# gattia/pyfocusr

Measured on AMD Instinct MI355X. Metric: lowest-k eigenpairs/sec + KNN-correspondence wall-clock, 250k-vertex mesh pair k=5, higher is better.
Workload: dtype f64

## Files before the change

### pyfocusr_amd/csrc/pf_eigs.hip

```cpp
#include <math.h>

#include <algorithm>
#include <vector>

#include "pf_internal.h"
#include "pf_krylov.h"
#include "pf_launch.h"

namespace {

struct DeviceOps final : pfk::Ops {
    pf_graph* g;
    explicit DeviceOps(pf_graph* graph) : g(graph) {}
    int64_t n() const override { return g->n; }
    int64_t n_isolated() const override { return g->n_isolated; }
    int32_t n_components() const override { return g->n_components; }
    int32_t n_oneway() const override { return g->n_oneway; }
    bool symmetric() const override { return g->is_symmetric; }
    double spectral_bound() const override { return g->spectral_bound; }
    int ws_ensure(int32_t slots) override { return pf_ws_ensure(g, slots); }
    int lock_nulls(int32_t op, int32_t* locked) override { return pf_lock_null_vectors(g, op, locked); }
    int orth_strict(bool on) override { return pf_orth_strict(g, on ? 1 : 0); }
    int orth_always_twice(bool on, bool strict_otherwise) override { return pf_orth_strict(g, on ? 2 : (strict_otherwise ? 1 : 0)); }
    int orth_device_passes(bool on) override { return pf_orth_device_passes(g, on ? 1 : 0); }
// ... 14 lines not shown
    }
    int combine2(int32_t src_first, int32_t m, const double* Y, int32_t k, int32_t dst_first, int32_t src_first2, int32_t dst_first2) override {
        return pf_combine2(g, src_first, m, Y, k, dst_first, src_first2, dst_first2);
    }
    int copy(int32_t src, int32_t dst, int32_t count) override { return pf_ws_copy(g, src, dst, count); }
    int spmv_multi(int32_t op, int32_t src_first, int32_t dst_first, int32_t count) override {
        return pf_spmv_multi(g, op, src_first, dst_first, count);
    }
    int gram(int32_t first_a, int32_t count_a, int32_t first_b, int32_t count_b, double* out) override {
        return pf_gram(g, first_a, count_a, first_b, count_b, out);
    }
    int resnorms(int32_t ax_first, int32_t x_first, const double* lam, int32_t count, double* out) override {
        return pf_resnorms(g, ax_first, x_first, lam, count, out);
    }
    int gram_begin(int32_t first_a, int32_t count_a, int32_t first_b, int32_t count_b, bool self_b) override {
        PF_TRY(pf_gram_begin(g, first_a, count_a, first_b, count_b, 0));
        return self_b ? pf_gram_begin(g, first_b, count_b, first_b, count_b, 1) : PF_OK;
    }
    bool orth_split(int32_t first2, int32_t split) override { return pf_orth_split(g, first2, split) == PF_OK; }
    int gram_end(double* out) override { return pf_small_end(g, out); }
    int resnorms_begin(int32_t ax_first, int32_t x_first, const double* lam, int32_t count) override {
        return pf_resnorms_begin(g, ax_first, x_first, lam, count);
    }
    int resnorms_end(double* out) override { return pf_small_end(g, out); }
    int orth_begin_pair(pfk::Ops& other, const int32_t* o) override {
        return pf_orth_begin2(g, o[0], o[1], o[2], o[3], static_cast<DeviceOps&>(other).g, o[4], o[5], o[6], o[7]);
    }
    int cheb_pair(pfk::Ops& other, const int32_t* ci, const double* cd) override {
        return pf_cheb2(g, ci[0], ci[1], ci[2], ci[3], cd[0], cd[1], cd[2], static_cast<DeviceOps&>(other).g, ci[4], ci[5], ci[6], ci[7], cd[3],
                        cd[4], cd[5]);
    }
    int orth_cheb_pair(pfk::Ops& other, const int32_t* orth, const int32_t* ci, const double* cd) override {
// ... 102 lines not shown
```

### pyfocusr_amd/csrc/pf_eigsort.hip

```cpp
#include <float.h>
#include <string.h>

#include <vector>

#include "pf_internal.h"

extern "C" int pf_knn1_blocks(pf_ctx* c, const double* ref_block, int64_t n_ref, int32_t ref_stride, const double* qry_block, int64_t n_qry,
                              int32_t qry_stride, int32_t d, const int32_t* col_ref, const double* scale_ref, const int32_t* col_qry,
                              const double* scale_qry, int64_t* idx_out, double* d2_out);

namespace {

constexpr int ES_SORT_THREADS = 1024;
constexpr int ES_MAX_SAMPLES = 16384;
constexpr int ES_RED_THREADS = 256;

__global__ __launch_bounds__(PF_BLOCK) void k_es_gather(const double* __restrict__ fin, int32_t fc, const double* __restrict__ pts,
                                                        const int64_t* __restrict__ rows, int64_t m, int32_t k,
                                                        const int32_t* __restrict__ col, const double* __restrict__ sign,
                                                        double* __restrict__ vals, double* __restrict__ raw) {
    const int64_t e = (int64_t)blockIdx.x * PF_BLOCK + threadIdx.x;
    if (e >= m * (k + 3)) return;
    const int64_t c = e / m, r = e - c * m;
    if (c < k) vals[c * m + r] = fin[rows[r] * fc + col[c]] * sign[c];
    else raw[r * 3 + (c - k)] = pts[rows[r] * 3 + (c - k)];
}

__global__ __launch_bounds__(ES_RED_THREADS) void k_es_minmax(const double* __restrict__ raw, int64_t m, double* __restrict__ lohi) {
    __shared__ double slo[ES_RED_THREADS], shi[ES_RED_THREADS];
    const int c = blockIdx.x;
    double lo = INFINITY, hi = -INFINITY;
    for (int64_t r = threadIdx.x; r < m; r += ES_RED_THREADS) {
        const double v = raw[r * 3 + c];
        lo = v < lo ? v : lo;
        hi = v > hi ? v : hi;
    }
    slo[threadIdx.x] = lo;
    shi[threadIdx.x] = hi;
    __syncthreads();
    for (int s = ES_RED_THREADS / 2; s > 0; s >>= 1) {
        if (threadIdx.x < s) {
            slo[threadIdx.x] = slo[threadIdx.x + s] < slo[threadIdx.x] ? slo[threadIdx.x + s] : slo[threadIdx.x];
            shi[threadIdx.x] = shi[threadIdx.x + s] > shi[threadIdx.x] ? shi[threadIdx.x + s] : shi[threadIdx.x];
        }
        __syncthreads();
    }
    if (threadIdx.x == 0) {
        lohi[c] = slo[0];
        lohi[3 + c] = shi[0];
    }
}

__global__ __launch_bounds__(PF_BLOCK) void k_es_normalize(const double* __restrict__ raw, const double* __restrict__ lohi, int64_t m,
                                                           double* __restrict__ out) {
    const int64_t e = (int64_t)blockIdx.x * PF_BLOCK + threadIdx.x;
    if (e >= m * 3) return;
    const int c = (int)(e % 3);
    out[e] = (raw[e] - lohi[c]) / (lohi[3 + c] - lohi[c]);
}

__global__ __launch_bounds__(ES_SORT_THREADS) void k_es_sort_log(const double* __restrict__ vals_t, const double* __restrict__ vals_s,
                                                                 int64_t mt, int64_t ms, int32_t k, double* __restrict__ lt,
                                                                 double* __restrict__ ls, double* __restrict__ lsf) {
    extern __shared__ double buf[];
    const int b = blockIdx.x;
    const int64_t m = b < k ? mt : ms;
    int n_pow2 = 2;
    while (n_pow2 < m) n_pow2 <<= 1;
    const double* src = b < k ? vals_t + (int64_t)b * m : vals_s + (int64_t)(b - k) * m;
    for (int i = threadIdx.x; i < n_pow2; i += ES_SORT_THREADS) buf[i] = i < m ? src[i] : INFINITY;
    __syncthreads();
    for (int size = 2; size <= n_pow2; size <<= 1) {
        for (int stride = size >> 1; stride > 0; stride >>= 1) {
            for (int t = threadIdx.x; t < n_pow2 / 2; t += ES_SORT_THREADS) {
                const int pos = 2 * t - (t & (stride - 1));
                const double a = buf[pos], c = buf[pos + stride];
                const bool up = (pos & size) == 0;
                if ((a > c) == up) {
                    buf[pos] = c;
                    buf[pos + stride] = a;
                }
            }
            __syncthreads();
        }
    }
    const double eps = DBL_EPSILON;
    if (b < k) {
        for (int64_t i = threadIdx.x; i < m; i += ES_SORT_THREADS) lt[(int64_t)b * m + i] = log(buf[i] + 0.5 + eps);
    } else {
        const int64_t o = (int64_t)(b - k) * m;
        for (int64_t i = threadIdx.x; i < m; i += ES_SORT_THREADS) {
            ls[o + i] = log(buf[i] + 0.5 + eps);
            lsf[o + i] = log(-buf[m - 1 - i] + 0.5 + eps);
        }
    }
}

__device__ __forceinline__ double es_block_sum(double v, double* sh) {
    sh[threadIdx.x] = v;
    __syncthreads();
    for (int s = ES_RED_THREADS / 2; s > 0; s >>= 1) {
        if (threadIdx.x < s) sh[threadIdx.x] += sh[threadIdx.x + s];
        __syncthreads();
    }
    const double r = sh[0];
    __syncthreads();
    return r;
}

// ... 12 lines not shown
            const double len = (double)(to - from) * unit;
            acc += len * fabs(t - ls[(int64_t)j * ms + b]);
            accf += len * fabs(t - lsf[(int64_t)j * ms + b]);
        }
    }
    acc = es_block_sum(acc, sh);
    accf = es_block_sum(accf, sh);
    if (threadIdx.x == 0) {
        out[i * k + j] = acc;
        out[k * k + i * k + j] = accf;
    }
}

__global__ __launch_bounds__(ES_RED_THREADS) void k_es_spatial(const double* __restrict__ vals_t, const double* __restrict__ vals_s,
                                                               const int64_t* __restrict__ idx, int64_t m, int64_t ms, int32_t k,
                                                               double* __restrict__ out) {
    __shared__ double sh[ES_RED_THREADS];
    const int i = blockIdx.x / k, j = blockIdx.x - i * k;
    double a = 0.0, f = 0.0;
    for (int64_t r = threadIdx.x; r < m; r += ES_RED_THREADS) {
        const int64_t nn = idx[r];
        const double t = vals_t[(int64_t)i * m + r], s = (nn >= 0 && nn < ms) ? vals_s[(int64_t)j * ms + nn] : NAN;
        const double d0 = s - t, d1 = -s - t;
        a += d0 * d0;
        f += d1 * d1;
    }
    a = es_block_sum(a, sh);
    f = es_block_sum(f, sh);
    if (threadIdx.x == 0) {
        out[2 * k * k + i * k + j] = sqrt(a) / (double)m;
        out[3 * k * k + i * k + j] = sqrt(f) / (double)m;
    }
}

}

// ... 24 lines not shown

    const size_t head = sizeof(int64_t) * (size_t)(mt + ms);
    const size_t small = ((sizeof(int32_t) * 2 * k + 7) & ~(size_t)7) + sizeof(double) * 2 * k;
    std::vector<unsigned char> host(head + small);
    memcpy(host.data(), rows_t, sizeof(int64_t) * (size_t)mt);
    memcpy(host.data() + sizeof(int64_t) * (size_t)mt, rows_s, sizeof(int64_t) * (size_t)ms);
    int32_t* hcol = reinterpret_cast<int32_t*>(host.data() + head);
    double* hsign = reinterpret_cast<double*>(host.data() + head + ((sizeof(int32_t) * 2 * k + 7) & ~(size_t)7));
    for (int32_t i = 0; i < k; ++i) {
        hcol[i] = col_t[i];
        hcol[k + i] = col_s[i];
        hsign[i] = sign_t[i];
        hsign[k + i] = sign_s[i];
    }
    const size_t kt = (size_t)k * (size_t)mt, ks = (size_t)k * (size_t)ms;
    const size_t doubles = 2 * kt + 3 * ks + 6 * (size_t)(mt + ms) + 12 + 4 * (size_t)k * k;
    unsigned char* d = nullptr;
    const size_t up_bytes = (host.size() + 7) & ~(size_t)7, out_bytes = sizeof(double) * 4 * (size_t)k * k;
    unsigned char* pin = nullptr;
    PF_TRY(pf_pinned_scratch(c, up_bytes + out_bytes, reinterpret_cast<void**>(&pin)));
    memcpy(pin, host.data(), host.size());
    PF_HIP(pf_malloc(st, (void**)&d, up_bytes + sizeof(double) * doubles));
    int rc = PF_OK;
    do {
        auto fail = [&](hipError_t e) {
            if (e == hipSuccess) return false;
            pf_set_error("pf_eigsort_costs: %s", hipGetErrorString(e));
            rc = PF_E_HIP;
            return true;
        };
        if ((rc = pf_copy_by_kernel(st, pin, d, up_bytes)) != PF_OK) break;
        const int64_t* d_rows_t = reinterpret_cast<const int64_t*>(d);
        const int64_t* d_rows_s = d_rows_t + mt;
        const int32_t* d_col = reinterpret_cast<const int32_t*>(d + head);
        const double* d_sign = reinterpret_cast<const double*>(d + head + ((sizeof(int32_t) * 2 * k + 7) & ~(size_t)7));
        double* base = reinterpret_cast<double*>(d + up_bytes);
        double* vals_t = base;
        double* vals_s = vals_t + kt;
        double* raw_t = vals_s + ks;
        double* raw_s = raw_t + 3 * mt;
        double* norm_t = raw_s + 3 * ms;
        double* norm_s = norm_t + 3 * mt;
        double* lohi = norm_s + 3 * ms;
        double* lt = lohi + 12;
        double* ls = lt + kt;
        double* lsf = ls + ks;
        double* d_out = lsf + ks;
        k_es_gather<<<pf_blocks(mt * (k + 3)), PF_BLOCK, 0, st>>>(gt->final_vecs, gt->final_count, gt->pts, d_rows_t, mt, k, d_col, d_sign,
                                                                  vals_t, raw_t);
        k_es_gather<<<pf_blocks(ms * (k + 3)), PF_BLOCK, 0, st>>>(gs->final_vecs, gs->final_count, gs->pts, d_rows_s, ms, k, d_col + k,
                                                                  d_sign + k, vals_s, raw_s);
        k_es_minmax<<<3, ES_RED_THREADS, 0, st>>>(raw_t, mt, lohi);
        k_es_minmax<<<3, ES_RED_THREADS, 0, st>>>(raw_s, ms, lohi + 6);
        k_es_normalize<<<pf_blocks(3 * mt), PF_BLOCK, 0, st>>>(raw_t, lohi, mt, norm_t);
        k_es_normalize<<<pf_blocks(3 * ms), PF_BLOCK, 0, st>>>(raw_s, lohi + 6, ms, norm_s);
        k_es_sort_log<<<(unsigned)(2 * k), ES_SORT_THREADS, sort_lds, st>>>(vals_t, vals_s, mt, ms, k, lt, ls, lsf);
        k_es_w1<<<(unsigned)(k * k), ES_RED_THREADS, 0, st>>>(lt, ls, lsf, mt, ms, k, d_out);
        if (fail(hipGetLastError())) break;
        const int32_t cols3[3] = {0, 1, 2};
        const double ones3[3] = {1.0, 1.0, 1.0};
        rc = pf_knn1_blocks(c, norm_s, ms, 3, norm_t, mt, 3, 3, cols3, ones3, cols3, ones3, idx_out, nullptr);
        if (rc != PF_OK) break;
        k_es_spatial<<<(unsigned)(k * k), ES_RED_THREADS, 0, st>>>(vals_t, vals_s, c->knn_idx.p, mt, ms, k, d_out);
        if (fail(hipGetLastError())) break;
        if ((rc = pf_copy_by_kernel(st, d_out, pin + up_bytes, out_bytes)) != PF_OK) break;
        if (fail(hipStreamSynchronize(st))) break;
        memcpy(out, pin + up_bytes, out_bytes);
    } while (0);
    if (rc != PF_OK) (void)hipStreamSynchronize(st);
    pf_free(st, d);
    return rc;
}
```

### pyfocusr_amd/csrc/pf_internal.h

```cpp
#pragma once
#include <hip/hip_runtime.h>
#include <stdint.h>
#include <atomic>
#include <map>
#include <mutex>
#include <type_traits>
#include <unordered_map>
#include <vector>

#include "../../include/pyfocusr_hip.h"
#include "pf_scratch.h"

void pf_set_error(const char* fmt, ...);

#define PF_HIP(call)                                                                          \
    do {                                                                                      \
        hipError_t e_ = (call);                                                               \
        if (e_ != hipSuccess) {                                                               \
            pf_set_error("%s:%d %s: %s", __FILE__, __LINE__, #call, hipGetErrorString(e_));   \
            (void)hipGetLastError();  \
            return PF_E_HIP;                                                                  \
        }                                                                                     \
    } while (0)

// ... 296 lines not shown

int pf_graph_finish_general(pf_graph* g, const double* d_pts);

int pf_exclusive_scan_i32(hipStream_t st, const int32_t* in, int32_t* out, int64_t n);
int pf_exclusive_scan_i64(hipStream_t st, const int64_t* in, int64_t* out, int64_t n);

int pf_reduce_ensure(pf_graph* g, int32_t count);

int pf_compute_order(pf_graph* g, const double* d_pts, int32_t* d_overflow = nullptr);
int pf_morton_order(pf_graph* g, const double* d_pts, int32_t* d_overflow);

static inline int32_t pf_window_rows(int64_t n_pad) { return n_pad <= 262144 ? 1024 : (n_pad <= 524288 ? 2048 : 4096); }

int pf_knn1_device(pf_ctx* c, const double* ref_block, int64_t n_ref, int32_t ref_stride, const double* qry_block, int64_t n_qry,
                   int32_t qry_stride, int32_t d);

int pf_knn_extent(hipStream_t st, const double* pts, int64_t n, int32_t d, unsigned long long* ext);

constexpr int PF_KNN_TREE_MIN_D = 7;
int pf_knn_tree_run(pf_ctx* c);

int pf_gram_begin(pf_graph* g, int32_t first_a, int32_t count_a, int32_t first_b, int32_t count_b, int32_t append);
int pf_resnorms_begin(pf_graph* g, int32_t ax_first, int32_t x_first, const double* lam, int32_t count);
int pf_small_end(pf_graph* g, double* out);
int pf_combine2(pf_graph* g, int32_t src_first, int32_t m, const double* Y, int32_t k, int32_t dst_first, int32_t src_first2,
                int32_t dst_first2);

struct pf_persist_args {
    pf_graph* g;
    const double* vals;
    const double* src;
    double* dst;
    int32_t degree;
    double c, e, rho;
};
int pf_persist_cheb(const pf_persist_args* a, const pf_persist_args* b , int* done, double* lds_bytes ,
                    bool first_try = true );
// ... 13 lines not shown
```

### pyfocusr_amd/csrc/pf_knn.hip

```cpp
#include <hipcub/hipcub.hpp>

#include <string.h>

#include <algorithm>

#include "pf_internal.h"
#include "pf_wave.h"

namespace {

constexpr int KNN_LDS_DOUBLES = 4096;

struct KnnGrid {
    int a0, a1;
    int r0, r1;
    double lo0, lo1;
    double s0, s1;
};

__device__ __forceinline__ int cell_of(double x, double lo, double scale, int r) {
    const double t = (x - lo) * scale;
    return t > 0.0 ? (t >= (double)r ? r - 1 : (int)t) : 0;
}

// ... 853 lines not shown
           int64_t* idx_out, double* d2_out) {
    PF_TRY(knn_upload_k(c, ref, n_ref, qry, n_qry, d, k));
    PF_TRY(pf_knn_run(c));
    return pf_knn_download(c, idx_out, d2_out);
}

int pf_knn1(pf_ctx* c, const double* ref, int64_t n_ref, const double* qry, int64_t n_qry, int32_t d, int64_t* idx_out,
            double* d2_out) {
    PF_TRY(pf_knn_upload(c, ref, n_ref, qry, n_qry, d));
    PF_TRY(pf_knn_run(c));
    return pf_knn_download(c, idx_out, d2_out);
}

static int knn1_blocks_run(pf_ctx* c, const double* ref_block, int64_t n_ref, int32_t ref_stride, const double* qry_block, int64_t n_qry,
                           int32_t qry_stride, int32_t d, const int32_t* col_ref, const double* scale_ref, const int32_t* col_qry,
                           const double* scale_qry) {
    PF_TRY(knn_prepare(c, n_ref, n_qry, d, 1));
    hipStream_t st = c->stream;
    CoordMap mr{}, mq{};
    for (int32_t k = 0; k < d; ++k) {
        mr.col[k] = col_ref[k], mr.scale[k] = scale_ref[k];
        mq.col[k] = col_qry[k], mq.scale[k] = scale_qry[k];
    }
    k_coords_from_final<<<pf_blocks(n_ref * d), PF_BLOCK, 0, st>>>(ref_block, n_ref, ref_stride, d, mr, c->knn_ref.p);
    k_coords_from_final<<<pf_blocks(n_qry * d), PF_BLOCK, 0, st>>>(qry_block, n_qry, qry_stride, d, mq, c->knn_qry.p);
    PF_HIP(hipGetLastError());
    c->knn_ready = true;
    return pf_knn_run(c);
}

int pf_knn1_blocks(pf_ctx* c, const double* ref_block, int64_t n_ref, int32_t ref_stride, const double* qry_block, int64_t n_qry,
                   int32_t qry_stride, int32_t d, const int32_t* col_ref, const double* scale_ref, const int32_t* col_qry,
                   const double* scale_qry, int64_t* idx_out, double* d2_out) {
    PF_CHECK(c && ref_block && qry_block && col_ref && scale_ref && col_qry && scale_qry && idx_out, PF_E_ARG,
             "pf_knn1_blocks: NULL argument");
    PF_CHECK(d >= 1 && d <= 16 && ref_stride >= 1 && qry_stride >= 1, PF_E_ARG, "pf_knn1_blocks: d = %d / strides out of range", d);
    for (int32_t k = 0; k < d; ++k)
        PF_CHECK(col_ref[k] >= 0 && col_ref[k] < ref_stride && col_qry[k] >= 0 && col_qry[k] < qry_stride, PF_E_ARG,
                 "pf_knn1_blocks: column %d out of range", k);
    PF_TRY(knn1_blocks_run(c, ref_block, n_ref, ref_stride, qry_block, n_qry, qry_stride, d, col_ref, scale_ref, col_qry, scale_qry));
    return pf_knn_download(c, idx_out, d2_out);
// ... 22 lines not shown
int pf_knn_extent(hipStream_t st, const double* pts, int64_t n, int32_t d, unsigned long long* ext) {
    PF_HIP(hipMemsetAsync(ext, 0xff, 16 * sizeof(unsigned long long), st));
    PF_HIP(hipMemsetAsync(ext + 16, 0x00, 16 * sizeof(unsigned long long), st));
    k_extent<<<256, PF_BLOCK, 0, st>>>(pts, n, d, ext);
    return PF_OK;
}

int pf_knn1_device(pf_ctx* c, const double* ref_block, int64_t n_ref, int32_t ref_stride, const double* qry_block, int64_t n_qry,
                   int32_t qry_stride, int32_t d) {
    PF_CHECK(c && ref_block && qry_block && d >= 1 && d <= 16 && d <= ref_stride && d <= qry_stride, PF_E_ARG, "pf_knn1_device: bad argument");
    int32_t col[16];
    double one[16];
    for (int32_t k = 0; k < 16; ++k) col[k] = k, one[k] = 1.0;
    return knn1_blocks_run(c, ref_block, n_ref, ref_stride, qry_block, n_qry, qry_stride, d, col, one, col, one);
}
```

### pyfocusr_amd/csrc/pf_operator.hip

```cpp
#include <math.h>
#include <stdlib.h>
#include <string.h>

#include <algorithm>
#include <atomic>
#include <map>
#include <mutex>
#include <vector>

#include "pf_internal.h"
#include "pf_launch.h"

namespace {

#ifndef PF_OP_BLOCK
#define PF_OP_BLOCK 256
#endif
struct OpArgs {
    const int64_t* slice_ptr;
    const int32_t* scol;
    const double* sval;
    const double* diag;
    const double* x;
    const double* prev;
// ... 635 lines not shown
    const int64_t lo = (int64_t)blockIdx.x * PF_DOT_CHUNK;
    const int64_t hi = lo + PF_DOT_CHUNK < n_pad ? lo + PF_DOT_CHUNK : n_pad;
    double s = 0.0;
    for (int64_t i = lo + threadIdx.x; i < hi; i += PF_BLOCK) {
        const double r = ax[i] - lam * x[i];
        s += r * r;
    }
#pragma unroll
    for (int off = PF_WAVE / 2; off > 0; off >>= 1) s += __shfl_down(s, off, PF_WAVE);
    if ((threadIdx.x & (PF_WAVE - 1)) == 0) red[threadIdx.x / PF_WAVE] = s;
    __syncthreads();
    if (threadIdx.x == 0) partial[blockIdx.x] = (red[0] + red[1]) + (red[2] + red[3]);
}

__global__ __launch_bounds__(PF_BLOCK) void k_gram_partial(const double* __restrict__ ws, int64_t n_pad, int32_t first_a, int32_t first_b,
                                                           int32_t count_b, int64_t n_chunks, double* __restrict__ partial) {
    __shared__ double red[PF_BLOCK / PF_WAVE];
    const int p = blockIdx.y;
    const int i = p / count_b, j = p - i * count_b;
    const double* v = ws + (int64_t)(first_b + j) * n_pad;
    const double* w = ws + (int64_t)(first_a + i) * n_pad;
    const int64_t lo = (int64_t)blockIdx.x * PF_DOT_CHUNK;
    const int64_t hi = lo + PF_DOT_CHUNK < n_pad ? lo + PF_DOT_CHUNK : n_pad;
    double s = 0.0;
    for (int64_t r = lo + 2 * threadIdx.x; r < hi; r += 2 * PF_BLOCK) {
        const double2 a = *reinterpret_cast<const double2*>(v + r);
        const double2 c = *reinterpret_cast<const double2*>(w + r);
        s += a.x * c.x;
        s += a.y * c.y;
    }
#pragma unroll
    for (int off = PF_WAVE / 2; off > 0; off >>= 1) s += __shfl_down(s, off, PF_WAVE);
    if ((threadIdx.x & (PF_WAVE - 1)) == 0) red[threadIdx.x / PF_WAVE] = s;
    __syncthreads();
    if (threadIdx.x == 0) partial[(int64_t)p * n_chunks + blockIdx.x] = (red[0] + red[1]) + (red[2] + red[3]);
}

constexpr int PF_RESNORMS_MAX = 64;
struct LamArgs {
    double lam[PF_RESNORMS_MAX];
};
__global__ __launch_bounds__(PF_BLOCK) void k_resnorms_partial(const double* __restrict__ ws, int64_t n_pad, int32_t ax_first,
                                                               int32_t x_first, LamArgs la, int64_t n_chunks,
                                                               double* __restrict__ partial) {
    __shared__ double red[PF_BLOCK / PF_WAVE];
    const int b = blockIdx.y;
    const double* ax = ws + (int64_t)(ax_first + b) * n_pad;
    const double* x = ws + (int64_t)(x_first + b) * n_pad;
    const double lam = la.lam[b];
    const int64_t lo = (int64_t)blockIdx.x * PF_DOT_CHUNK;
// ... 72 lines not shown
}

__global__ __launch_bounds__(PF_WAVE) void k_vec_stats_finish(const VecStats* __restrict__ partial, int64_t n_chunks,
                                                              VecStats* __restrict__ out) {
    const int b = blockIdx.x;
    VecStats st{0.0, INFINITY, -INFINITY, -1.0, 0.0, (int64_t)1 << 62};
    for (int64_t k = threadIdx.x; k < n_chunks; k += PF_WAVE) stats_merge(st, partial[(int64_t)b * n_chunks + k]);
#pragma unroll
    for (int off = PF_WAVE / 2; off > 0; off >>= 1) {
        VecStats o = stats_shfl(st, off);
        stats_merge(st, o);
    }
    if (threadIdx.x == 0) out[b] = st;
}

__global__ void k_vec_params(const VecStats* __restrict__ fin, int32_t count, int32_t minmax, double* __restrict__ params) {
    for (int c = threadIdx.x; c < count; c += blockDim.x) {
        const VecStats s = fin[c];
        const double sgn = s.at_absmax < 0.0 ? -1.0 : 1.0;
        const double scale = sgn / sqrt(s.sumsq);
        const double vmin = (sgn > 0 ? s.vmin : s.vmax) * scale;
        const double vmax = (sgn > 0 ? s.vmax : s.vmin) * scale;
        params[4 * c + 0] = scale;
        params[4 * c + 1] = minmax ? vmin : 0.0;
        params[4 * c + 2] = minmax ? (vmax - vmin) : 0.0;
        params[4 * c + 3] = minmax ? 0.5 : 0.0;
    }
}

__global__ __launch_bounds__(PF_BLOCK) void k_vec_apply(const double* __restrict__ ws, int64_t n_pad, int64_t n,
                                                        int32_t first, int32_t count, const double* __restrict__ sg,
                                                        const int32_t* __restrict__ iperm, const int32_t* __restrict__ mrank,
                                                        int32_t from_sym, const double* __restrict__ params, double* __restrict__ out) {
// ... 936 lines not shown
            } else {
                for (int i = 0; i < PF_STAGE_SLOTS; ++i) ctx->stage_ev[i] = nullptr;
            }
        }
        if (ctx->stage_ring) {
            const int slot = ctx->stage_next;
            ctx->stage_next = (slot + 1) % PF_STAGE_SLOTS;
            bool ok = true;
            if (!ctx->stage_ev[slot]) ok = hipEventCreateWithFlags(&ctx->stage_ev[slot], hipEventDisableTiming) == hipSuccess;
            else ok = hipEventSynchronize(ctx->stage_ev[slot]) == hipSuccess;
            if (ok) {
                void* dst = static_cast<unsigned char*>(ctx->stage_ring) + (size_t)slot * PF_STAGE_BYTES;
                memcpy(dst, Y, bytes);
                src = dst;
                staged = true;
                hipError_t es = hipMemcpyAsync(dY, src, bytes, hipMemcpyHostToDevice, st);
                if (es == hipSuccess) es = hipEventRecord(ctx->stage_ev[slot], st);
                if (es != hipSuccess) {
                    pf_free(st, dY);
                    PF_HIP(es);
                }
            } else {
                (void)hipGetLastError();
            }
        }
    }
    hipError_t e = staged ? hipSuccess : hipMemcpyAsync(dY, Y, bytes, hipMemcpyHostToDevice, st);
    for (int32_t c0 = 0; c0 < k && e == hipSuccess; c0 += COMBINE_COLS) {
        const int32_t nc = std::min(COMBINE_COLS, k - c0);
        k_combine<<<dim3(pf_blocks(g->n_pad), two ? 2u : 1u), PF_BLOCK, 0, st>>>(g->ws, g->n_pad, src_first, m, dY, k, c0, nc, dst_first, src_first2,
                                                                          dst_first2);
// ... 20 lines not shown
    PF_HIP(hipGetLastError());
    double r2 = 0.0;
    PF_HIP(hipMemcpyAsync(&r2, g->coef, sizeof(double), hipMemcpyDeviceToHost, st));
    PF_HIP(hipStreamSynchronize(st));
    *out = sqrt(r2 > 0.0 ? r2 : 0.0);
    return PF_OK;
}

int pf_gram(pf_graph* g, int32_t first_a, int32_t count_a, int32_t first_b, int32_t count_b, double* out) {
    PF_TRY(check_slots(g, first_a, count_a, "pf_gram"));
    PF_TRY(check_slots(g, first_b, count_b, "pf_gram"));
    PF_CHECK(out != nullptr && count_a > 0 && count_b > 0, PF_E_ARG, "pf_gram: bad argument");
    PF_TRY(pf_reduce_ensure(g, count_a * count_b));
    hipStream_t st = g->ctx->stream;
    k_gram_partial<<<dim3((unsigned)g->n_chunks, (unsigned)(count_a * count_b)), PF_BLOCK, 0, st>>>(g->ws, g->n_pad, first_a, first_b, count_b,
                                                                                                 g->n_chunks, g->partials);
    PF_HIP(hipGetLastError());
    k_dot_finish<<<(unsigned)(count_a * count_b), PF_WAVE, 0, st>>>(g->partials, g->n_chunks, g->coef, nullptr, 0);
    PF_HIP(hipGetLastError());
    return small_to_host(g, g->coef, out, (size_t)count_a * count_b);
}

}

static int small_begin(pf_graph* g, const double* d_src, size_t count, bool root, bool append = false) {
    PF_CHECK(append ? g->small_pending > 0 && !g->small_root && !root : g->small_pending == 0, PF_E_STATE,
             "pf_gram_begin / pf_resnorms_begin: a previous result has not been collected");
    pf_ctx* c = g->ctx;
    hipStream_t st = c->stream;
    const size_t offset = append ? (size_t)g->small_pending : 0;
    if (append) {
        PF_CHECK((int64_t)(offset + count) <= g->small_host_cap, PF_E_STATE, "pf_gram_begin: no room to append");
    } else if ((int64_t)(2 * count) > g->small_host_cap || !g->small_host) {
        if (g->small_host) {
            PF_HIP(hipStreamSynchronize(st));
            c->pinned_pool.emplace_back(g->small_host_cap, g->small_host);
            g->small_host = nullptr;
        }
        const int32_t cap = std::max((int32_t)(2 * count), 128);
        for (size_t i = 0; i < c->pinned_pool.size(); ++i)
            if (c->pinned_pool[i].first >= cap) {
                g->small_host_cap = c->pinned_pool[i].first;
                g->small_host = c->pinned_pool[i].second;
                c->pinned_pool.erase(c->pinned_pool.begin() + (long)i);
                break;
            }
        if (!g->small_host) {
            PF_HIP(hipHostMalloc((void**)&g->small_host, sizeof(double) * (size_t)(cap + 2), hipHostMallocDefault));
            g->small_host_cap = cap;
        }
    }
    if (!g->small_ev) {
        if (!c->event_pool.empty()) {
            g->small_ev = c->event_pool.back();
            c->event_pool.pop_back();
        } else {
            PF_HIP(hipEventCreateWithFlags(&g->small_ev, hipEventDisableTiming));
        }
    }
    PF_TRY(pf_copy_by_kernel(st, d_src, g->small_host + offset, sizeof(double) * count));
    PF_HIP(hipEventRecord(g->small_ev, st));
    g->small_pending = (int32_t)(offset + count);
    g->small_root = root;
    return PF_OK;
}

int pf_small_end(pf_graph* g, double* out) {
    PF_CHECK(g != nullptr && out != nullptr && g->small_pending > 0, PF_E_STATE, "pf_small_end: nothing to collect");
    PF_HIP(hipEventSynchronize(g->small_ev));
    const int32_t count = g->small_pending;
    g->small_pending = 0;
    for (int32_t i = 0; i < count; ++i) {
        const double v = g->small_host[i];
        out[i] = g->small_root ? sqrt(v > 0.0 ? v : 0.0) : v;
    }
    return PF_OK;
}

int pf_gram_begin(pf_graph* g, int32_t first_a, int32_t count_a, int32_t first_b, int32_t count_b, int32_t append) {
    PF_TRY(check_slots(g, first_a, count_a, "pf_gram"));
    PF_TRY(check_slots(g, first_b, count_b, "pf_gram"));
    PF_CHECK(count_a > 0 && count_b > 0, PF_E_ARG, "pf_gram: bad argument");
    PF_TRY(pf_reduce_ensure(g, count_a * count_b));
    hipStream_t st = g->ctx->stream;
    k_gram_partial<<<dim3((unsigned)g->n_chunks, (unsigned)(count_a * count_b)), PF_BLOCK, 0, st>>>(g->ws, g->n_pad, first_a, first_b, count_b,
                                                                                                 g->n_chunks, g->partials);
    PF_HIP(hipGetLastError());
    k_dot_finish<<<(unsigned)(count_a * count_b), PF_WAVE, 0, st>>>(g->partials, g->n_chunks, g->coef, nullptr, 0);
    PF_HIP(hipGetLastError());
    return small_begin(g, g->coef, (size_t)count_a * count_b, false, append != 0);
}

int pf_resnorms_begin(pf_graph* g, int32_t ax_first, int32_t x_first, const double* lam, int32_t count) {
    PF_TRY(check_slots(g, ax_first, count, "pf_resnorms"));
    PF_TRY(check_slots(g, x_first, count, "pf_resnorms"));
    PF_CHECK(lam != nullptr && count > 0, PF_E_ARG, "pf_resnorms: bad argument");
    hipStream_t st = g->ctx->stream;
    PF_TRY(pf_reduce_ensure(g, count));
    for (int32_t at = 0; at < count; at += PF_RESNORMS_MAX) {
        const int32_t nb = std::min(count - at, PF_RESNORMS_MAX);
        LamArgs la{};
        for (int32_t i = 0; i < nb; ++i) la.lam[i] = lam[at + i];
        k_resnorms_partial<<<dim3((unsigned)g->n_chunks, (unsigned)nb), PF_BLOCK, 0, st>>>(g->ws, g->n_pad, ax_first + at, x_first + at, la,
                                                                                        g->n_chunks, g->partials);
        PF_HIP(hipGetLastError());
        k_dot_finish<<<(unsigned)nb, PF_WAVE, 0, st>>>(g->partials, g->n_chunks, g->coef + at, nullptr, 0);
        PF_HIP(hipGetLastError());
    }
    return small_begin(g, g->coef, (size_t)count, true);
}

extern "C" {

int pf_resnorms(pf_graph* g, int32_t ax_first, int32_t x_first, const double* lam, int32_t count, double* out) {
    PF_TRY(check_slots(g, ax_first, count, "pf_resnorms"));
    PF_TRY(check_slots(g, x_first, count, "pf_resnorms"));
    PF_CHECK(out != nullptr && lam != nullptr && count > 0, PF_E_ARG, "pf_resnorms: bad argument");
    hipStream_t st = g->ctx->stream;
    PF_TRY(pf_reduce_ensure(g, count));
    for (int32_t at = 0; at < count; at += PF_RESNORMS_MAX) {
        const int32_t nb = std::min(count - at, PF_RESNORMS_MAX);
        LamArgs la{};
        for (int32_t i = 0; i < nb; ++i) la.lam[i] = lam[at + i];
        k_resnorms_partial<<<dim3((unsigned)g->n_chunks, (unsigned)nb), PF_BLOCK, 0, st>>>(g->ws, g->n_pad, ax_first + at, x_first + at, la,
// ... 103 lines not shown
    VecStats* part = reinterpret_cast<VecStats*>(g->partials);
    VecStats* fin = part + (size_t)count * g->n_chunks;
    dim3 grid((unsigned)g->n_chunks, (unsigned)count);
    k_vec_stats_partial<<<grid, PF_BLOCK, 0, st>>>(g->ws, g->n_pad, g->n, first, g->sg, g->perm, g->perm_m, from_sym, g->n_chunks, part);
    PF_HIP(hipGetLastError());
    k_vec_stats_finish<<<(unsigned)count, PF_WAVE, 0, st>>>(part, g->n_chunks, fin);
    PF_HIP(hipGetLastError());
    double *d_params = nullptr, *d_out = nullptr;
    pf_free(st, g->final_vecs);
    g->final_vecs = nullptr;
    g->final_count = 0;
    PF_HIP(pf_malloc(st, (void**)&d_params, sizeof(double) * 4 * (size_t)count + sizeof(VecStats) * (size_t)count));
    VecStats* d_stats = reinterpret_cast<VecStats*>(d_params + 4 * (size_t)count);
    hipError_t e = pf_malloc(st, (void**)&d_out, sizeof(double) * (size_t)g->n * count);
    if (e == hipSuccess) {
        k_vec_params<<<1, PF_WAVE, 0, st>>>(fin, count, minmax, d_params);
        k_vec_apply<<<pf_blocks(g->n), PF_BLOCK, 0, st>>>(g->ws, g->n_pad, g->n, first, count, g->sg, g->iperm, g->mrank, from_sym, d_params, d_out);
        e = hipGetLastError();
    }
    if (e == hipSuccess) e = hipMemcpyAsync(d_stats, fin, sizeof(VecStats) * count, hipMemcpyDeviceToDevice, st);
    if (e == hipSuccess) e = hipEventRecord(g->final_ready, st);
    if (e == hipSuccess) e = hipStreamWaitEvent(ctx->copy_stream, g->final_ready, 0);
    if (e == hipSuccess) e = hipMemcpyAsync(g->final_stats, d_stats, sizeof(VecStats) * count, hipMemcpyDeviceToHost, ctx->copy_stream);
    if (e == hipSuccess) e = hipEventRecord(g->final_done, ctx->copy_stream);
    if (e != hipSuccess) {
        (void)hipStreamSynchronize(ctx->copy_stream);
        pf_free(st, d_params);
        pf_free(st, d_out);
        PF_HIP(e);
    }
    g->final_vecs = d_out;
    g->final_count = count;
    g->final_params = d_params;
    g->final_pending = count;
    g->final_check = count;
// ... 372 lines not shown
```

Before: 1022.

## Batch eigsort launches, overlap sort on side stream, fuse gram and small-result copies

```diff
diff --git a/pyfocusr_amd/csrc/pf_eigs.hip b/pyfocusr_amd/csrc/pf_eigs.hip
--- a/pyfocusr_amd/csrc/pf_eigs.hip
+++ b/pyfocusr_amd/csrc/pf_eigs.hip
@@ -52,8 +52,7 @@
         return pf_resnorms(g, ax_first, x_first, lam, count, out);
     }
     int gram_begin(int32_t first_a, int32_t count_a, int32_t first_b, int32_t count_b, bool self_b) override {
-        PF_TRY(pf_gram_begin(g, first_a, count_a, first_b, count_b, 0));
-        return self_b ? pf_gram_begin(g, first_b, count_b, first_b, count_b, 1) : PF_OK;
+        return pf_gram_begin(g, first_a, count_a, first_b, count_b, self_b ? 1 : 0);
     }
     bool orth_split(int32_t first2, int32_t split) override { return pf_orth_split(g, first2, split) == PF_OK; }
     int gram_end(double* out) override { return pf_small_end(g, out); }
diff --git a/pyfocusr_amd/csrc/pf_eigsort.hip b/pyfocusr_amd/csrc/pf_eigsort.hip
--- a/pyfocusr_amd/csrc/pf_eigsort.hip
+++ b/pyfocusr_amd/csrc/pf_eigsort.hip
@@ -4,10 +4,6 @@
 #include <vector>
 
 #include "pf_internal.h"
-
-extern "C" int pf_knn1_blocks(pf_ctx* c, const double* ref_block, int64_t n_ref, int32_t ref_stride, const double* qry_block, int64_t n_qry,
-                              int32_t qry_stride, int32_t d, const int32_t* col_ref, const double* scale_ref, const int32_t* col_qry,
-                              const double* scale_qry, int64_t* idx_out, double* d2_out);
 
 namespace {
 
@@ -15,19 +11,35 @@
 constexpr int ES_MAX_SAMPLES = 16384;
 constexpr int ES_RED_THREADS = 256;
 
-__global__ __launch_bounds__(PF_BLOCK) void k_es_gather(const double* __restrict__ fin, int32_t fc, const double* __restrict__ pts,
-                                                        const int64_t* __restrict__ rows, int64_t m, int32_t k,
-                                                        const int32_t* __restrict__ col, const double* __restrict__ sign,
-                                                        double* __restrict__ vals, double* __restrict__ raw) {
+struct EsSet {
+    const double* fin;
+    const double* pts;
+    const int64_t* rows;
+    const int32_t* col;
+    const double* sign;
+    double* vals;
+    double* raw;
+    double* norm;
+    double* lohi;
+    int64_t m;
+    int32_t fc;
+};
+
+__global__ __launch_bounds__(PF_BLOCK) void k_es_gather(EsSet t, EsSet s, int32_t k) {
+    const EsSet& a = blockIdx.y ? s : t;
+    const int64_t m = a.m;
     const int64_t e = (int64_t)blockIdx.x * PF_BLOCK + threadIdx.x;
     if (e >= m * (k + 3)) return;
     const int64_t c = e / m, r = e - c * m;
-    if (c < k) vals[c * m + r] = fin[rows[r] * fc + col[c]] * sign[c];
-    else raw[r * 3 + (c - k)] = pts[rows[r] * 3 + (c - k)];
-}
-
-__global__ __launch_bounds__(ES_RED_THREADS) void k_es_minmax(const double* __restrict__ raw, int64_t m, double* __restrict__ lohi) {
+    if (c < k) a.vals[c * m + r] = a.fin[a.rows[r] * a.fc + a.col[c]] * a.sign[c];
+    else a.raw[r * 3 + (c - k)] = a.pts[a.rows[r] * 3 + (c - k)];
+}
+
+__global__ __launch_bounds__(ES_RED_THREADS) void k_es_minmax(EsSet t, EsSet s) {
     __shared__ double slo[ES_RED_THREADS], shi[ES_RED_THREADS];
+    const EsSet& a = blockIdx.y ? s : t;
+    const double* __restrict__ raw = a.raw;
+    const int64_t m = a.m;
     const int c = blockIdx.x;
     double lo = INFINITY, hi = -INFINITY;
     for (int64_t r = threadIdx.x; r < m; r += ES_RED_THREADS) {
@@ -38,25 +50,97 @@
     slo[threadIdx.x] = lo;
     shi[threadIdx.x] = hi;
     __syncthreads();
-    for (int s = ES_RED_THREADS / 2; s > 0; s >>= 1) {
-        if (threadIdx.x < s) {
-            slo[threadIdx.x] = slo[threadIdx.x + s] < slo[threadIdx.x] ? slo[threadIdx.x + s] : slo[threadIdx.x];
-            shi[threadIdx.x] = shi[threadIdx.x + s] > shi[threadIdx.x] ? shi[threadIdx.x + s] : shi[threadIdx.x];
+    for (int s2 = ES_RED_THREADS / 2; s2 > 0; s2 >>= 1) {
+        if (threadIdx.x < s2) {
+            slo[threadIdx.x] = slo[threadIdx.x + s2] < slo[threadIdx.x] ? slo[threadIdx.x + s2] : slo[threadIdx.x];
+            shi[threadIdx.x] = shi[threadIdx.x + s2] > shi[threadIdx.x] ? shi[threadIdx.x + s2] : shi[threadIdx.x];
         }
         __syncthreads();
     }
     if (threadIdx.x == 0) {
-        lohi[c] = slo[0];
-        lohi[3 + c] = shi[0];
-    }
-}
-
-__global__ __launch_bounds__(PF_BLOCK) void k_es_normalize(const double* __restrict__ raw, const double* __restrict__ lohi, int64_t m,
-                                                           double* __restrict__ out) {
+        a.lohi[c] = slo[0];
+        a.lohi[3 + c] = shi[0];
+    }
+}
+
+__global__ __launch_bounds__(PF_BLOCK) void k_es_normalize(EsSet t, EsSet s) {
+    const EsSet& a = blockIdx.y ? s : t;
     const int64_t e = (int64_t)blockIdx.x * PF_BLOCK + threadIdx.x;
-    if (e >= m * 3) return;
+    if (e >= a.m * 3) return;
     const int c = (int)(e % 3);
-    out[e] = (raw[e] - lohi[c]) / (lohi[3 + c] - lohi[c]);
+    a.norm[e] = (a.raw[e] - a.lohi[c]) / (a.lohi[3 + c] - a.lohi[c]);
+}
+
+template <int E>
+__device__ __forceinline__ void es_sort_log(const double* __restrict__ src, int64_t m, int n_pow2, double* buf, double* __restrict__ out,
+                                            double* __restrict__ out_flip) {
+    const int t = threadIdx.x, lane = t & (PF_WAVE - 1);
+    const int base = t * E;
+    const bool active = base < n_pow2;
+    double v[E];
+#pragma unroll
+    for (int e = 0; e < E; ++e) v[e] = base + e < m ? src[base + e] : INFINITY;
+    for (int size = 2; size <= n_pow2; size <<= 1) {
+        int stride = size >> 1;
+        if (stride >= PF_WAVE * E) {
+            if (active) {
+#pragma unroll
+                for (int e = 0; e < E; ++e) buf[base + e] = v[e];
+            }
+            __syncthreads();
+            for (; stride >= PF_WAVE * E; stride >>= 1) {
+                for (int p = t; p < n_pow2 / 2; p += ES_SORT_THREADS) {
+                    const int pos = 2 * p - (p & (stride - 1));
+                    const double a = buf[pos], c = buf[pos + stride];
+                    const bool up = (pos & size) == 0;
+                    if ((a > c) == up) {
+                        buf[pos] = c;
+                        buf[pos + stride] = a;
+                    }
+                }
+                __syncthreads();
+            }
+            if (active) {
+#pragma unroll
+                for (int e = 0; e < E; ++e) v[e] = buf[base + e];
+            }
+        }
+        const bool up = (base & size) == 0;
+        for (; stride >= E; stride >>= 1) {
+            const int lm = stride / E;
+            const bool lower = (lane & lm) == 0;
+#pragma unroll
+            for (int e = 0; e < E; ++e) {
+                const double other = __shfl_xor(v[e], lm, PF_WAVE);
+                const double a = lower ? v[e] : other, c = lower ? other : v[e];
+                if ((a > c) == up) v[e] = other;
+            }
+        }
+#pragma unroll
+        for (int s = E / 2; s > 0; s >>= 1) {
+            if (s < size) {
+#pragma unroll
+                for (int e = 0; e < E; ++e) {
+                    if ((e & s) == 0) {
+                        const double a = v[e], c = v[e + s];
+                        if ((a > c) == (((base + e) & size) == 0)) {
+                            v[e] = c;
+                            v[e + s] = a;
+                        }
+                    }
+                }
+            }
+        }
+    }
+    const double eps = DBL_EPSILON;
+#pragma unroll
+    for (int e = 0; e < E; ++e) {
+        const int64_t pos = base + e;
+        if (pos < m) {
+            out[pos] = log(v[e] + 0.5 + eps);
+            if (out_flip) out_flip[m - 1 - pos] = log(-v[e] + 0.5 + eps);
+        }
+    }
 }
 
 __global__ __launch_bounds__(ES_SORT_THREADS) void k_es_sort_log(const double* __restrict__ vals_t, const double* __restrict__ vals_s,
@@ -68,31 +152,15 @@
     int n_pow2 = 2;
     while (n_pow2 < m) n_pow2 <<= 1;
     const double* src = b < k ? vals_t + (int64_t)b * m : vals_s + (int64_t)(b - k) * m;
-    for (int i = threadIdx.x; i < n_pow2; i += ES_SORT_THREADS) buf[i] = i < m ? src[i] : INFINITY;
-    __syncthreads();
-    for (int size = 2; size <= n_pow2; size <<= 1) {
-        for (int stride = size >> 1; stride > 0; stride >>= 1) {
-            for (int t = threadIdx.x; t < n_pow2 / 2; t += ES_SORT_THREADS) {
-                const int pos = 2 * t - (t & (stride - 1));
-                const double a = buf[pos], c = buf[pos + stride];
-                const bool up = (pos & size) == 0;
-                if ((a > c) == up) {
-                    buf[pos] = c;
-                    buf[pos + stride] = a;
-                }
-            }
-            __syncthreads();
-        }
-    }
-    const double eps = DBL_EPSILON;
-    if (b < k) {
-        for (int64_t i = threadIdx.x; i < m; i += ES_SORT_THREADS) lt[(int64_t)b * m + i] = log(buf[i] + 0.5 + eps);
-    } else {
-        const int64_t o = (int64_t)(b - k) * m;
-        for (int64_t i = threadIdx.x; i < m; i += ES_SORT_THREADS) {
-            ls[o + i] = log(buf[i] + 0.5 + eps);
-            lsf[o + i] = log(-buf[m - 1 - i] + 0.5 + eps);
-        }
+    double* out = b < k ? lt + (int64_t)b * m : ls + (int64_t)(b - k) * m;
+    double* out_flip = b < k ? nullptr : lsf + (int64_t)(b - k) * m;
+    switch (n_pow2 / ES_SORT_THREADS) {
+        case 0:
+        case 1: es_sort_log<1>(src, m, n_pow2, buf, out, out_flip); break;
+        case 2: es_sort_log<2>(src, m, n_pow2, buf, out, out_flip); break;
+        case 4: es_sort_log<4>(src, m, n_pow2, buf, out, out_flip); break;
+        case 8: es_sort_log<8>(src, m, n_pow2, buf, out, out_flip); break;
+        default: es_sort_log<ES_MAX_SAMPLES / ES_SORT_THREADS>(src, m, n_pow2, buf, out, out_flip); break;
     }
 }
 
@@ -135,12 +203,13 @@
 
 __global__ __launch_bounds__(ES_RED_THREADS) void k_es_spatial(const double* __restrict__ vals_t, const double* __restrict__ vals_s,
                                                                const int64_t* __restrict__ idx, int64_t m, int64_t ms, int32_t k,
-                                                               double* __restrict__ out) {
+                                                               double* __restrict__ out, int64_t* __restrict__ idx_copy) {
     __shared__ double sh[ES_RED_THREADS];
     const int i = blockIdx.x / k, j = blockIdx.x - i * k;
     double a = 0.0, f = 0.0;
     for (int64_t r = threadIdx.x; r < m; r += ES_RED_THREADS) {
         const int64_t nn = idx[r];
+        if (blockIdx.x == 0) idx_copy[r] = nn;
         const double t = vals_t[(int64_t)i * m + r], s = (nn >= 0 && nn < ms) ? vals_s[(int64_t)j * ms + nn] : NAN;
         const double d0 = s - t, d1 = -s - t;
         a += d0 * d0;
@@ -195,60 +264,75 @@
         hsign[k + i] = sign_s[i];
     }
     const size_t kt = (size_t)k * (size_t)mt, ks = (size_t)k * (size_t)ms;
-    const size_t doubles = 2 * kt + 3 * ks + 6 * (size_t)(mt + ms) + 12 + 4 * (size_t)k * k;
+    const size_t doubles = 2 * kt + 3 * ks + 6 * (size_t)(mt + ms) + 12 + 4 * (size_t)k * k + (size_t)mt;
     unsigned char* d = nullptr;
-    const size_t up_bytes = (host.size() + 7) & ~(size_t)7, out_bytes = sizeof(double) * 4 * (size_t)k * k;
+    const size_t up_bytes = (host.size() + 7) & ~(size_t)7, cost_bytes = sizeof(double) * 4 * (size_t)k * k;
+    const size_t out_bytes = cost_bytes + sizeof(int64_t) * (size_t)mt;
     unsigned char* pin = nullptr;
     PF_TRY(pf_pinned_scratch(c, up_bytes + out_bytes, reinterpret_cast<void**>(&pin)));
     memcpy(pin, host.data(), host.size());
+    hipStream_t sb = pf_stream_b(c);
     PF_HIP(pf_malloc(st, (void**)&d, up_bytes + sizeof(double) * doubles));
     int rc = PF_OK;
+    bool forked = false;
     do {
         auto fail = [&](hipError_t e) {
             if (e == hipSuccess) return false;
             pf_set_error("pf_eigsort_costs: %s", hipGetErrorString(e));
+            (void)hipGetLastError();
             rc = PF_E_HIP;
             return true;
         };
         if ((rc = pf_copy_by_kernel(st, pin, d, up_bytes)) != PF_OK) break;
         const int64_t* d_rows_t = reinterpret_cast<const int64_t*>(d);
-        const int64_t* d_rows_s = d_rows_t + mt;
         const int32_t* d_col = reinterpret_cast<const int32_t*>(d + head);
         const double* d_sign = reinterpret_cast<const double*>(d + head + ((sizeof(int32_t) * 2 * k + 7) & ~(size_t)7));
         double* base = reinterpret_cast<double*>(d + up_bytes);
-        double* vals_t = base;
-        double* vals_s = vals_t + kt;
-        double* raw_t = vals_s + ks;
-        double* raw_s = raw_t + 3 * mt;
-        double* norm_t = raw_s + 3 * ms;
-        double* norm_s = norm_t + 3 * mt;
-        double* lohi = norm_s + 3 * ms;
-        double* lt = lohi + 12;
+        EsSet T{}, S{};
+        T.fin = gt->final_vecs, T.fc = gt->final_count, T.pts = gt->pts, T.rows = d_rows_t, T.col = d_col, T.sign = d_sign, T.m = mt;
+        S.fin = gs->final_vecs, S.fc = gs->final_count, S.pts = gs->pts, S.rows = d_rows_t + mt, S.col = d_col + k, S.sign = d_sign + k, S.m = ms;
+        T.vals = base;
+        S.vals = T.vals + kt;
+        T.raw = S.vals + ks;
+        S.raw = T.raw + 3 * mt;
+        T.norm = S.raw + 3 * ms;
+        S.norm = T.norm + 3 * mt;
+        T.lohi = S.norm + 3 * ms;
+        S.lohi = T.lohi + 6;
+        double* lt = T.lohi + 12;
         double* ls = lt + kt;
         double* lsf = ls + ks;
         double* d_out = lsf + ks;
-        k_es_gather<<<pf_blocks(mt * (k + 3)), PF_BLOCK, 0, st>>>(gt->final_vecs, gt->final_count, gt->pts, d_rows_t, mt, k, d_col, d_sign,
-                                                                  vals_t, raw_t);
-        k_es_gather<<<pf_blocks(ms * (k + 3)), PF_BLOCK, 0, st>>>(gs->final_vecs, gs->final_count, gs->pts, d_rows_s, ms, k, d_col + k,
-                                                                  d_sign + k, vals_s, raw_s);
-        k_es_minmax<<<3, ES_RED_THREADS, 0, st>>>(raw_t, mt, lohi);
-        k_es_minmax<<<3, ES_RED_THREADS, 0, st>>>(raw_s, ms, lohi + 6);
-        k_es_normalize<<<pf_blocks(3 * mt), PF_BLOCK, 0, st>>>(raw_t, lohi, mt, norm_t);
-        k_es_normalize<<<pf_blocks(3 * ms), PF_BLOCK, 0, st>>>(raw_s, lohi + 6, ms, norm_s);
-        k_es_sort_log<<<(unsigned)(2 * k), ES_SORT_THREADS, sort_lds, st>>>(vals_t, vals_s, mt, ms, k, lt, ls, lsf);
-        k_es_w1<<<(unsigned)(k * k), ES_RED_THREADS, 0, st>>>(lt, ls, lsf, mt, ms, k, d_out);
+        int64_t* d_idx = reinterpret_cast<int64_t*>(d_out + 4 * (size_t)k * k);
+        const int64_t m_max = mt > ms ? mt : ms;
+        k_es_gather<<<dim3(pf_blocks(m_max * (k + 3)), 2), PF_BLOCK, 0, st>>>(T, S, k);
         if (fail(hipGetLastError())) break;
-        const int32_t cols3[3] = {0, 1, 2};
-        const double ones3[3] = {1.0, 1.0, 1.0};
-        rc = pf_knn1_blocks(c, norm_s, ms, 3, norm_t, mt, 3, 3, cols3, ones3, cols3, ones3, idx_out, nullptr);
-        if (rc != PF_OK) break;
-        k_es_spatial<<<(unsigned)(k * k), ES_RED_THREADS, 0, st>>>(vals_t, vals_s, c->knn_idx.p, mt, ms, k, d_out);
+        hipStream_t sh = st;
+        if (sb) {
+            if (fail(hipEventRecord(c->fork_ev, st)) || fail(hipStreamWaitEvent(sb, c->fork_ev, 0))) break;
+            forked = true;
+            sh = sb;
+        }
+        k_es_sort_log<<<(unsigned)(2 * k), ES_SORT_THREADS, sort_lds, sh>>>(T.vals, S.vals, mt, ms, k, lt, ls, lsf);
+        k_es_w1<<<(unsigned)(k * k), ES_RED_THREADS, 0, sh>>>(lt, ls, lsf, mt, ms, k, d_out);
         if (fail(hipGetLastError())) break;
+        if (forked && fail(hipEventRecord(c->join_ev, sb))) break;
+        k_es_minmax<<<dim3(3, 2), ES_RED_THREADS, 0, st>>>(T, S);
+        k_es_normalize<<<dim3(pf_blocks(3 * m_max), 2), PF_BLOCK, 0, st>>>(T, S);
+        if (fail(hipGetLastError())) break;
+        if ((rc = pf_knn1_queue(c, S.norm, ms, 3, T.norm, mt, 3, 3)) != PF_OK) break;
+        k_es_spatial<<<(unsigned)(k * k), ES_RED_THREADS, 0, st>>>(T.vals, S.vals, c->knn_idx.p, mt, ms, k, d_out, d_idx);
+        if (fail(hipGetLastError())) break;
+        if (forked && fail(hipStreamWaitEvent(st, c->join_ev, 0))) break;
         if ((rc = pf_copy_by_kernel(st, d_out, pin + up_bytes, out_bytes)) != PF_OK) break;
         if (fail(hipStreamSynchronize(st))) break;
-        memcpy(out, pin + up_bytes, out_bytes);
+        memcpy(out, pin + up_bytes, cost_bytes);
+        memcpy(idx_out, pin + up_bytes + cost_bytes, sizeof(int64_t) * (size_t)mt);
     } while (0);
-    if (rc != PF_OK) (void)hipStreamSynchronize(st);
+    if (rc != PF_OK) {
+        (void)hipStreamSynchronize(st);
+        if (forked) (void)hipStreamSynchronize(sb);
+    }
     pf_free(st, d);
     return rc;
 }
diff --git a/pyfocusr_amd/csrc/pf_internal.h b/pyfocusr_amd/csrc/pf_internal.h
--- a/pyfocusr_amd/csrc/pf_internal.h
+++ b/pyfocusr_amd/csrc/pf_internal.h
@@ -334,13 +334,15 @@
 
 int pf_knn1_device(pf_ctx* c, const double* ref_block, int64_t n_ref, int32_t ref_stride, const double* qry_block, int64_t n_qry,
                    int32_t qry_stride, int32_t d);
+int pf_knn1_queue(pf_ctx* c, const double* ref_block, int64_t n_ref, int32_t ref_stride, const double* qry_block, int64_t n_qry,
+                  int32_t qry_stride, int32_t d);
 
 int pf_knn_extent(hipStream_t st, const double* pts, int64_t n, int32_t d, unsigned long long* ext);
 
 constexpr int PF_KNN_TREE_MIN_D = 7;
 int pf_knn_tree_run(pf_ctx* c);
 
-int pf_gram_begin(pf_graph* g, int32_t first_a, int32_t count_a, int32_t first_b, int32_t count_b, int32_t append);
+int pf_gram_begin(pf_graph* g, int32_t first_a, int32_t count_a, int32_t first_b, int32_t count_b, int32_t self_b);
 int pf_resnorms_begin(pf_graph* g, int32_t ax_first, int32_t x_first, const double* lam, int32_t count);
 int pf_small_end(pf_graph* g, double* out);
 int pf_combine2(pf_graph* g, int32_t src_first, int32_t m, const double* Y, int32_t k, int32_t dst_first, int32_t src_first2,
diff --git a/pyfocusr_amd/csrc/pf_knn.hip b/pyfocusr_amd/csrc/pf_knn.hip
--- a/pyfocusr_amd/csrc/pf_knn.hip
+++ b/pyfocusr_amd/csrc/pf_knn.hip
@@ -891,7 +891,7 @@
 
 static int knn1_blocks_run(pf_ctx* c, const double* ref_block, int64_t n_ref, int32_t ref_stride, const double* qry_block, int64_t n_qry,
                            int32_t qry_stride, int32_t d, const int32_t* col_ref, const double* scale_ref, const int32_t* col_qry,
-                           const double* scale_qry) {
+                           const double* scale_qry, bool queue_only = false) {
     PF_TRY(knn_prepare(c, n_ref, n_qry, d, 1));
     hipStream_t st = c->stream;
     CoordMap mr{}, mq{};
@@ -902,6 +902,7 @@
     k_coords_from_final<<<pf_blocks(n_ref * d), PF_BLOCK, 0, st>>>(ref_block, n_ref, ref_stride, d, mr, c->knn_ref.p);
     k_coords_from_final<<<pf_blocks(n_qry * d), PF_BLOCK, 0, st>>>(qry_block, n_qry, qry_stride, d, mq, c->knn_qry.p);
     PF_HIP(hipGetLastError());
+    if (queue_only) return knn_search(c);
     c->knn_ready = true;
     return pf_knn_run(c);
 }
@@ -954,3 +955,12 @@
     for (int32_t k = 0; k < 16; ++k) col[k] = k, one[k] = 1.0;
     return knn1_blocks_run(c, ref_block, n_ref, ref_stride, qry_block, n_qry, qry_stride, d, col, one, col, one);
 }
+
+int pf_knn1_queue(pf_ctx* c, const double* ref_block, int64_t n_ref, int32_t ref_stride, const double* qry_block, int64_t n_qry,
+                  int32_t qry_stride, int32_t d) {
+    PF_CHECK(c && ref_block && qry_block && d >= 1 && d <= 16 && d <= ref_stride && d <= qry_stride, PF_E_ARG, "pf_knn1_queue: bad argument");
+    int32_t col[16];
+    double one[16];
+    for (int32_t k = 0; k < 16; ++k) col[k] = k, one[k] = 1.0;
+    return knn1_blocks_run(c, ref_block, n_ref, ref_stride, qry_block, n_qry, qry_stride, d, col, one, col, one, true);
+}
diff --git a/pyfocusr_amd/csrc/pf_operator.hip b/pyfocusr_amd/csrc/pf_operator.hip
--- a/pyfocusr_amd/csrc/pf_operator.hip
+++ b/pyfocusr_amd/csrc/pf_operator.hip
@@ -673,9 +673,13 @@
 }
 
 __global__ __launch_bounds__(PF_BLOCK) void k_gram_partial(const double* __restrict__ ws, int64_t n_pad, int32_t first_a, int32_t first_b,
-                                                           int32_t count_b, int64_t n_chunks, double* __restrict__ partial) {
+                                                           int32_t count_b, int64_t n_chunks, double* __restrict__ partial, int32_t split) {
     __shared__ double red[PF_BLOCK / PF_WAVE];
-    const int p = blockIdx.y;
+    int p = blockIdx.y;
+    if (p >= split) {
+        p -= split;
+        first_a = first_b;
+    }
     const int i = p / count_b, j = p - i * count_b;
     const double* v = ws + (int64_t)(first_b + j) * n_pad;
     const double* w = ws + (int64_t)(first_a + i) * n_pad;
@@ -692,7 +696,7 @@
     for (int off = PF_WAVE / 2; off > 0; off >>= 1) s += __shfl_down(s, off, PF_WAVE);
     if ((threadIdx.x & (PF_WAVE - 1)) == 0) red[threadIdx.x / PF_WAVE] = s;
     __syncthreads();
-    if (threadIdx.x == 0) partial[(int64_t)p * n_chunks + blockIdx.x] = (red[0] + red[1]) + (red[2] + red[3]);
+    if (threadIdx.x == 0) partial[(int64_t)blockIdx.y * n_chunks + blockIdx.x] = (red[0] + red[1]) + (red[2] + red[3]);
 }
 
 constexpr int PF_RESNORMS_MAX = 64;
@@ -795,9 +799,11 @@
     if (threadIdx.x == 0) out[b] = st;
 }
 
-__global__ void k_vec_params(const VecStats* __restrict__ fin, int32_t count, int32_t minmax, double* __restrict__ params) {
+__global__ void k_vec_params(const VecStats* __restrict__ fin, int32_t count, int32_t minmax, double* __restrict__ params,
+                             VecStats* __restrict__ keep) {
     for (int c = threadIdx.x; c < count; c += blockDim.x) {
         const VecStats s = fin[c];
+        keep[c] = s;
         const double sgn = s.at_absmax < 0.0 ? -1.0 : 1.0;
         const double scale = sgn / sqrt(s.sumsq);
         const double vmin = (sgn > 0 ? s.vmin : s.vmax) * scale;
@@ -1764,7 +1770,7 @@
                 memcpy(dst, Y, bytes);
                 src = dst;
                 staged = true;
-                hipError_t es = hipMemcpyAsync(dY, src, bytes, hipMemcpyHostToDevice, st);
+                hipError_t es = pf_copy_by_kernel(st, src, dY, bytes) == PF_OK ? hipSuccess : hipErrorUnknown;
                 if (es == hipSuccess) es = hipEventRecord(ctx->stage_ev[slot], st);
                 if (es != hipSuccess) {
                     pf_free(st, dY);
@@ -1815,7 +1821,7 @@
     PF_TRY(pf_reduce_ensure(g, count_a * count_b));
     hipStream_t st = g->ctx->stream;
     k_gram_partial<<<dim3((unsigned)g->n_chunks, (unsigned)(count_a * count_b)), PF_BLOCK, 0, st>>>(g->ws, g->n_pad, first_a, first_b, count_b,
-                                                                                                 g->n_chunks, g->partials);
+                                                                                                 g->n_chunks, g->partials, count_a * count_b);
     PF_HIP(hipGetLastError());
     k_dot_finish<<<(unsigned)(count_a * count_b), PF_WAVE, 0, st>>>(g->partials, g->n_chunks, g->coef, nullptr, 0);
     PF_HIP(hipGetLastError());
@@ -1824,21 +1830,16 @@
 
 }
 
-static int small_begin(pf_graph* g, const double* d_src, size_t count, bool root, bool append = false) {
-    PF_CHECK(append ? g->small_pending > 0 && !g->small_root && !root : g->small_pending == 0, PF_E_STATE,
-             "pf_gram_begin / pf_resnorms_begin: a previous result has not been collected");
+static int small_place(pf_graph* g, size_t count, double** dst) {
+    PF_CHECK(g->small_pending == 0, PF_E_STATE, "pf_gram_begin / pf_resnorms_begin: a previous result has not been collected");
     pf_ctx* c = g->ctx;
-    hipStream_t st = c->stream;
-    const size_t offset = append ? (size_t)g->small_pending : 0;
-    if (append) {
-        PF_CHECK((int64_t)(offset + count) <= g->small_host_cap, PF_E_STATE, "pf_gram_begin: no room to append");
-    } else if ((int64_t)(2 * count) > g->small_host_cap || !g->small_host) {
+    if ((int64_t)count > g->small_host_cap || !g->small_host) {
         if (g->small_host) {
-            PF_HIP(hipStreamSynchronize(st));
+            PF_HIP(hipStreamSynchronize(c->stream));
             c->pinned_pool.emplace_back(g->small_host_cap, g->small_host);
             g->small_host = nullptr;
         }
-        const int32_t cap = std::max((int32_t)(2 * count), 128);
+        const int32_t cap = std::max((int32_t)count, 128);
         for (size_t i = 0; i < c->pinned_pool.size(); ++i)
             if (c->pinned_pool[i].first >= cap) {
                 g->small_host_cap = c->pinned_pool[i].first;
@@ -1859,9 +1860,13 @@
             PF_HIP(hipEventCreateWithFlags(&g->small_ev, hipEventDisableTiming));
         }
     }
-    PF_TRY(pf_copy_by_kernel(st, d_src, g->small_host + offset, sizeof(double) * count));
-    PF_HIP(hipEventRecord(g->small_ev, st));
-    g->small_pending = (int32_t)(offset + count);
+    *dst = g->small_host;
+    return PF_OK;
+}
+
+static int small_record(pf_graph* g, size_t count, bool root) {
+    PF_HIP(hipEventRecord(g->small_ev, g->ctx->stream));
+    g->small_pending = (int32_t)count;
     g->small_root = root;
     return PF_OK;
 }
@@ -1878,18 +1883,22 @@
     return PF_OK;
 }
 
-int pf_gram_begin(pf_graph* g, int32_t first_a, int32_t count_a, int32_t first_b, int32_t count_b, int32_t append) {
+int pf_gram_begin(pf_graph* g, int32_t first_a, int32_t count_a, int32_t first_b, int32_t count_b, int32_t self_b) {
     PF_TRY(check_slots(g, first_a, count_a, "pf_gram"));
     PF_TRY(check_slots(g, first_b, count_b, "pf_gram"));
     PF_CHECK(count_a > 0 && count_b > 0, PF_E_ARG, "pf_gram: bad argument");
-    PF_TRY(pf_reduce_ensure(g, count_a * count_b));
+    const int32_t split = count_a * count_b, total = split + (self_b ? count_b * count_b : 0);
+    PF_CHECK(total <= 65535, PF_E_ARG, "pf_gram: %d pairs in one launch", total);
+    PF_TRY(pf_reduce_ensure(g, total));
+    double* dst = nullptr;
+    PF_TRY(small_place(g, (size_t)total, &dst));
     hipStream_t st = g->ctx->stream;
-    k_gram_partial<<<dim3((unsigned)g->n_chunks, (unsigned)(count_a * count_b)), PF_BLOCK, 0, st>>>(g->ws, g->n_pad, first_a, first_b, count_b,
-                                                                                                 g->n_chunks, g->partials);
-    PF_HIP(hipGetLastError());
-    k_dot_finish<<<(unsigned)(count_a * count_b), PF_WAVE, 0, st>>>(g->partials, g->n_chunks, g->coef, nullptr, 0);
-    PF_HIP(hipGetLastError());
-    return small_begin(g, g->coef, (size_t)count_a * count_b, false, append != 0);
+    k_gram_partial<<<dim3((unsigned)g->n_chunks, (unsigned)total), PF_BLOCK, 0, st>>>(g->ws, g->n_pad, first_a, first_b, count_b, g->n_chunks,
+                                                                                   g->partials, split);
+    PF_HIP(hipGetLastError());
+    k_dot_finish<<<(unsigned)total, PF_WAVE, 0, st>>>(g->partials, g->n_chunks, dst, nullptr, 0);
+    PF_HIP(hipGetLastError());
+    return small_record(g, (size_t)total, false);
 }
 
 int pf_resnorms_begin(pf_graph* g, int32_t ax_first, int32_t x_first, const double* lam, int32_t count) {
@@ -1898,6 +1907,8 @@
     PF_CHECK(lam != nullptr && count > 0, PF_E_ARG, "pf_resnorms: bad argument");
     hipStream_t st = g->ctx->stream;
     PF_TRY(pf_reduce_ensure(g, count));
+    double* dst = nullptr;
+    PF_TRY(small_place(g, (size_t)count, &dst));
     for (int32_t at = 0; at < count; at += PF_RESNORMS_MAX) {
         const int32_t nb = std::min(count - at, PF_RESNORMS_MAX);
         LamArgs la{};
@@ -1905,10 +1916,10 @@
         k_resnorms_partial<<<dim3((unsigned)g->n_chunks, (unsigned)nb), PF_BLOCK, 0, st>>>(g->ws, g->n_pad, ax_first + at, x_first + at, la,
                                                                                         g->n_chunks, g->partials);
         PF_HIP(hipGetLastError());
-        k_dot_finish<<<(unsigned)nb, PF_WAVE, 0, st>>>(g->partials, g->n_chunks, g->coef + at, nullptr, 0);
+        k_dot_finish<<<(unsigned)nb, PF_WAVE, 0, st>>>(g->partials, g->n_chunks, dst + at, nullptr, 0);
         PF_HIP(hipGetLastError());
     }
-    return small_begin(g, g->coef, (size_t)count, true);
+    return small_record(g, (size_t)count, true);
 }
 
 extern "C" {
@@ -2042,11 +2053,10 @@
     VecStats* d_stats = reinterpret_cast<VecStats*>(d_params + 4 * (size_t)count);
     hipError_t e = pf_malloc(st, (void**)&d_out, sizeof(double) * (size_t)g->n * count);
     if (e == hipSuccess) {
-        k_vec_params<<<1, PF_WAVE, 0, st>>>(fin, count, minmax, d_params);
+        k_vec_params<<<1, PF_WAVE, 0, st>>>(fin, count, minmax, d_params, d_stats);
         k_vec_apply<<<pf_blocks(g->n), PF_BLOCK, 0, st>>>(g->ws, g->n_pad, g->n, first, count, g->sg, g->iperm, g->mrank, from_sym, d_params, d_out);
         e = hipGetLastError();
     }
-    if (e == hipSuccess) e = hipMemcpyAsync(d_stats, fin, sizeof(VecStats) * count, hipMemcpyDeviceToDevice, st);
     if (e == hipSuccess) e = hipEventRecord(g->final_ready, st);
     if (e == hipSuccess) e = hipStreamWaitEvent(ctx->copy_stream, g->final_ready, 0);
     if (e == hipSuccess) e = hipMemcpyAsync(g->final_stats, d_stats, sizeof(VecStats) * count, hipMemcpyDeviceToHost, ctx->copy_stream);
```

Measured after the change: 1037, median of 6. 1.5% higher.
